# l90lpa/fv3-jedi-linearmodel

Hardware: AMD Instinct MI355X
Metric: column-updates/s per TL+AD dyn step (higher is better)
Workload: dtype f64; 1 GPU; C192L127 hydrostatic TL+AD, six cube faces dealt over 1 GPU(s) (6 per rank), table-driven exchange (221184 columns per GPU), k_split=2 n_split=6 dt=450s nq=4, hord mt/vt/tm/dp/tr=2/2/2/2/2 (sponge: 1/1/1/1 below level 9), kord=17, nord=1; columns_per_gpu=221184

## Files before the change

### fv3_jedi_linearmodel_amd/csrc/dycore.h

```cpp
#pragma once
#include "../../include/fv3lm.h"
#include "stages.h"
#include "column.h"
#include "exchange.h"
#include "nh.h"
#include "nh_ad.h"
#include "tpfused.h"
#include "tpad.h"
#include "tp2.h"
#include "dampt.h"
#include <functional>
#include <map>
#include <memory>
#include <set>
#include <string>
#include <vector>

namespace fv3 {

#ifdef FV3LM_HOST_EMUL
inline void* dev_alloc(size_t n) { void* p = std::calloc(n ? n : 1, 1); return p; }
inline void dev_free(void* p) { std::free(p); }
inline void dev_zero(Exec&, void* p, size_t n) { std::memset(p, 0, n); }
inline void dev_copy(Exec&, void* d, const void* s, size_t n) { std::memcpy(d, s, n); }
inline void h2d(Exec&, void* d, const void* s, size_t n) { std::memcpy(d, s, n); }
inline void d2h(Exec&, void* d, const void* s, size_t n) { std::memcpy(d, s, n); }
inline void dev_sync(Exec&) {}
#else
#define HIPCHK(x) do { hipError_t e_ = (x); if (e_ != hipSuccess) { char b_[320]; std::snprintf(b_, sizeof b_, "HIP error '%s' at %s:%d (%s)", hipGetErrorString(e_), __FILE__, __LINE__, #x); set_sticky(b_); } } while (0)
inline void* dev_alloc(size_t n) {
  void* p = nullptr;
  if (!sticky_error().empty()) return nullptr;
  const hipError_t e = hipMalloc(&p, n ? n : 8);
  if (e != hipSuccess) { char b_[200]; std::snprintf(b_, sizeof b_, "hipMalloc of %zu bytes failed: %s", n, hipGetErrorString(e)); set_sticky(b_); (void)hipGetLastError(); return nullptr; }
  HIPCHK(hipMemset(p, 0, n ? n : 8));
  return p;
}
inline void dev_free(void* p) { if (p) (void)hipFree(p); }
__global__ void __launch_bounds__(256) k_zero16(double2* p, size_t n2) {
  const size_t stride = (size_t)gridDim.x * 256;
  for (size_t i = (size_t)blockIdx.x * 256 + threadIdx.x; i < n2; i += stride) p[i] = make_double2(0., 0.);
}
inline void dev_zero(Exec& ex, void* p, size_t n) {
  if (n >= ((size_t)1 << 20) && ((uintptr_t)p & 7) == 0) {
    char* q = (char*)p;
    if ((uintptr_t)q & 15) { HIPCHK(hipMemsetAsync(q, 0, 8, ex.stream)); q += 8; n -= 8; }
    const size_t n2 = n / 16, want = (n2 + 255) / 256;
    hipLaunchKernelGGL(k_zero16, dim3((unsigned)(want < 8192 ? want : 8192)), dim3(256), 0, ex.stream, (double2*)q, n2);
    if (n & 15) HIPCHK(hipMemsetAsync(q + n2 * 16, 0, n & 15, ex.stream));
    return;
  }
  HIPCHK(hipMemsetAsync(p, 0, n, ex.stream));
}
inline void dev_copy(Exec& ex, void* d, const void* s, size_t n) { HIPCHK(hipMemcpyAsync(d, s, n, hipMemcpyDeviceToDevice, ex.stream)); }
inline void h2d(Exec& ex, void* d, const void* s, size_t n) { HIPCHK(hipMemcpyAsync(d, s, n, hipMemcpyHostToDevice, ex.stream)); HIPCHK(hipStreamSynchronize(ex.stream)); }
inline void d2h(Exec& ex, void* d, const void* s, size_t n) { HIPCHK(hipMemcpyAsync(d, s, n, hipMemcpyDeviceToHost, ex.stream)); HIPCHK(hipStreamSynchronize(ex.stream)); }
inline void dev_sync(Exec& ex) { HIPCHK(hipStreamSynchronize(ex.stream)); }
#endif

struct Arena {
  double* t = nullptr; double* p = nullptr; size_t cap = 0, used = 0;
  void measure() { cap = (size_t)1 << 56; t = p = (double*)(uintptr_t)4096; used = 0; }
  void init(size_t ndoubles) { cap = ndoubles; t = (double*)dev_alloc(cap * 8); p = (double*)dev_alloc(cap * 8); used = 0; }
  void destroy() { dev_free(t); dev_free(p); t = p = nullptr; }
  Fld take(size_t n, int nk) {
    if (used + n > cap) { set_sticky("internal sizing error: field arena overflow"); Fld f; f.t = t; f.p = p; f.nk = nk; return f; }
    Fld f; f.t = t + used; f.p = p + used; f.nk = nk; used += n; return f;
  }
};

typedef fv3lm_options Options;

inline bool resolve_level(const Options& o, int k, int npz, LevelParams& lp) {
  int hord_m = o.hord_mt, hord_t = o.hord_tm, hord_v = o.hord_vt, hord_p = o.hord_dp;
  int nord_k = o.nord, nord_v = (2 > o.nord) ? o.nord : 2;
  double d2_divg = (0.20 > o.d2_bg) ? o.d2_bg : 0.20;
  double damp_vt = o.do_vort_damp ? o.vtdm4 : 0.;
  int nord_w = nord_v, nord_t = nord_v;
  double damp_w = damp_vt, damp_t = damp_vt, d_con_k = o.d_con;
  if (npz == 1 || o.n_sponge < 0) {
    d2_divg = o.d2_bg;
  } else if (k == 1) {
    nord_k = 0;
    if (0.01 < o.d2_bg) d2_divg = (o.d2_bg < o.d2_bg_k1) ? o.d2_bg_k1 : o.d2_bg;
    else if (0.01 < o.d2_bg_k1) d2_divg = o.d2_bg_k1;
    else d2_divg = 0.01;
    nord_w = 0; damp_w = d2_divg;
    if (o.do_vort_damp) { nord_v = 0; damp_vt = 0.5 * d2_divg; }
    d_con_k = 0.;
  } else {
    const int max1 = (2 < o.n_sponge - 1) ? o.n_sponge - 1 : 2;
    if (k == max1 && o.d2_bg_k2 > 0.01) {
      nord_k = 0; d2_divg = (o.d2_bg < o.d2_bg_k2) ? o.d2_bg_k2 : o.d2_bg;
      nord_w = 0; damp_w = d2_divg;
      if (o.do_vort_damp) { nord_v = 0; damp_vt = 0.5 * d2_divg; }
      d_con_k = 0.;
    } else {
      const int max2 = (3 < o.n_sponge) ? o.n_sponge : 3;
      if (k == max2 && o.d2_bg_k2 > 0.05) {
        nord_k = 0; d2_divg = (o.d2_bg < 0.2 * o.d2_bg_k2) ? 0.2 * o.d2_bg_k2 : o.d2_bg;
        nord_w = 0; damp_w = d2_divg; d_con_k = 0.;
      }
    }
  }
  int hmp = o.hord_mt_pert, htp = o.hord_tm_pert, hvp = o.hord_vt_pert, hpp = o.hord_dp_pert;
  int nord_k_pert = o.nord_pert;
  int nord_v_pert = (2 > o.nord_pert) ? o.nord_pert : 2;
  double damp_vt_pert = o.do_vort_damp_pert ? o.vtdm4_pert : 0.;
  double d2_divg_pert = (0.20 > o.d2_bg_pert) ? o.d2_bg_pert : 0.20;
  const int nord_t_pert = nord_v_pert; const double damp_t_pert = damp_vt_pert;
  if (k <= o.n_sponge_pert) {
    nord_k_pert = 0;
    if (k <= o.n_sponge_pert - 1) {
      if (o.hord_ks_traj) { hord_m = o.hord_mt_ks_traj; hord_t = o.hord_tm_ks_traj; hord_v = o.hord_vt_ks_traj; hord_p = o.hord_dp_ks_traj; }
      if (o.hord_ks_pert) { hmp = o.hord_mt_ks_pert; htp = o.hord_tm_ks_pert; hvp = o.hord_vt_ks_pert; hpp = o.hord_dp_ks_pert; }
    }
    const double kfac = (k == 1) ? o.d2_bg_k1_pert : (k == 2) ? o.d2_bg_k2_pert : o.d2_bg_ks_pert;
    double d2p;
    if (0.01 < o.d2_bg_pert) d2p = (o.d2_bg_pert < kfac) ? kfac : o.d2_bg_pert;
    else if (0.01 < kfac) d2p = kfac;
    else d2p = 0.01;
    d2_divg_pert = d2p;
    if (o.do_vort_damp_pert) { nord_v_pert = 0; damp_vt_pert = 0.5 * d2p; }
  }
  lp.hord_mt = hmp; lp.hord_vt = hvp; lp.hord_tm = htp; lp.hord_dp = hpp; lp.hord_tr = o.hord_tr_pert;
  lp.hord_tm_g = o.hord_tm_pert;
  lp.hord_mt_t = hord_m; lp.hord_vt_t = hord_v; lp.hord_tm_t = hord_t; lp.hord_dp_t = hord_p; lp.hord_tr_t = o.hord_tr; lp.hord_tm_g_t = o.hord_tm;
  lp.nord = nord_k; lp.nord_v = nord_v; lp.nord_w = nord_w; lp.nord_t = nord_t; lp.nord_v_pert = nord_v_pert;
  lp.d2_divg = d2_divg; lp.damp_vt = damp_vt; lp.damp_w = damp_w; lp.damp_t = damp_t; lp.d_con = d_con_k;
  lp.damp_vt_pert = damp_vt_pert;
  lp.split_damp = o.split_damp ? 1 : 0; lp.nord_t_pert = nord_t_pert; lp.damp_t_pert = damp_t_pert;
  lp.dddmp = o.dddmp; lp.d4_bg = o.d4_bg;
  if (o.split_damp) { lp.nord_p = nord_k_pert; lp.d2_divg_p = d2_divg_pert; lp.dddmp_p = o.dddmp_pert; lp.d4_bg_p = o.d4_bg_pert; }
  else { lp.nord_p = nord_k; lp.d2_divg_p = d2_divg; lp.dddmp_p = o.dddmp; lp.d4_bg_p = o.d4_bg; }
  return true;
}

struct Op {
  std::string group;
  std::function<void(Exec&, int)> fn;
  bool accum = false;
  unsigned modes = 7u;
  std::vector<double*> ad_in, ad_out;
  std::vector<int> ad_in_slot;
  std::function<void(unsigned, Rect)> set_wmask;
  std::vector<Rect> ad_out_rect;
  std::vector<double*> ad_store;
  std::string name;
  bool global = false;
  Op() = default;
  Op(std::string g_, std::function<void(Exec&, int)> f_, bool acc_ = false) : group(std::move(g_)), fn(std::move(f_)), accum(acc_) {}
};
typedef std::vector<Op> Program;
struct Progs {
  std::vector<Program> c; const int* cur = nullptr;
  Program& now() { return c[(size_t)(*cur < 0 ? 0 : *cur)]; }
  operator Program&() { return now(); }
  void clear() { now().clear(); }
};

struct Dycore {
  Geom g{}; Options opt; Exec ex; Ctx ctx{};
  double bdt = 0; int n_split = 1, k_split = 1, nq = 0;
// ... 210 lines not shown
      for (size_t n = 0; n < it->ad_in.size(); ++n) {
        double* q_ = it->ad_in[n];
        if (!inA(q_) || written.count(q_)) continue;
        const char* skip = std::getenv("FV3LM_AD_WRITE_SKIP");
        const bool skipped = skip && ("," + std::string(skip) + ",").find("," + it->name + ",") != std::string::npos;
        if (std::getenv("FV3LM_AD_WRITE_LIST") && it->set_wmask && !skipped && !zero.count(q_)) std::fprintf(stderr, "write-mode %s input %d\n", it->name.c_str(), it->ad_in_slot[n]);
        if (!off && !skipped && it->set_wmask && n < it->ad_in_slot.size() && !zero.count(q_)) {
          w |= 1u << it->ad_in_slot[n];
          grow((everywhere.count(q_) || !prod.count(q_)) ? whole : prod[q_]);
        }
        else zero.insert(q_);
        written.insert(q_);
      }
      if (it->set_wmask) it->set_wmask(w, wr);
    }
    std::vector<std::pair<double*, size_t>> out;
    for (double* q_ : zero) {
      const size_t n = size.count(q_) ? size[q_] : 0;
      if (!n) { set_sticky("internal error: adjoint plan met an unregistered work array"); continue; }
      if (!out.empty() && out.back().first + out.back().second == q_) out.back().second += n; else out.push_back({q_, n});
    }
    if (std::getenv("FV3LM_AD_WRITE_LIST")) { size_t tot = 0; for (auto& z_ : out) tot += z_.second; std::fprintf(stderr, "plan_adjoint: %zu work adjoints cleared per pass (%zu ranges, %.1f field-equivalents of %zu in the arena)\n", zero.size(), out.size(), double(tot) / double(n3 ? n3 : 1), size.size()); }
    return out;
  }
  std::vector<std::pair<double*, size_t>> acoustic_zero;

  void build_tp(Program& P, const char* grp, const std::string& pre, Fld q, Fld crx, Fld cry, Fld xfx, Fld yfx, Fld rax,
                Fld ray, Fld mx, Fld my, Fld mass, int hsel, int dsel, bool use_mass, Fld fx, Fld fy, int nk = 0, const Fld* acc4 = nullptr) {
    const int is = g.is(), ie = g.ie(), js = g.js(), je = g.je(), isd = g.isd(), ied = g.ied(), jsd = g.jsd(), jed = g.jed(), npz = nk ? nk : g.npz;
    const char* fenv = std::getenv("FV3LM_TP_FUSED");
    const bool fused = !(fenv && fenv[0] == '0');
    const char* aenv = std::getenv("FV3LM_TP_AD_FUSED");
    const int adf = !fused ? 0 : aenv ? (aenv[0] == '0' ? 0 : aenv[0] == '1' ? 1 : 2) : 2;
    const bool own_fo = adf == 0, own_mid = adf < 2;
    Fld fy2 = own_mid ? W((pre + "_fy2").c_str(), npz) : fy, q_i = own_mid ? W((pre + "_qi").c_str(), npz) : fx;
    Fld fx2 = own_mid ? W((pre + "_fx2").c_str(), npz) : fx, q_j = own_mid ? W((pre + "_qj").c_str(), npz) : fy;
    Fld fxo = own_fo ? W((pre + "_fxo").c_str(), npz) : fx2, fyo = own_fo ? W((pre + "_fyo").c_str(), npz) : fy2;
    const size_t first_op = P.size();
    auto ppm_y = [&](Fld qq, Fld out, Rect r, int cdir) {
      TpPpmY_<false> a; a.in[0] = qq; a.in[1] = cry; a.out[0] = out; a.k1 = npz; a.hsel = hsel;
      if (!g.face) { a.orect[0] = r; add(P, grp, a); return; }
      const int npy = g.ny + 1;
      a.orect[0] = isect(r, R(r.i0, r.i1, 4, npy - 3));
      TpPpmY_<true> e; e.in[0] = qq; e.in[1] = cry; e.out[0] = out; e.k1 = npz; e.hsel = hsel; e.cdir = cdir;
      std::vector<TpPpmY_<true>> ev;
      for (const Rect& er : {isect(r, R(r.i0, r.i1, r.j0, 3)), isect(r, R(r.i0, r.i1, npy - 2, r.j1))}) if (!is_empty(er)) { e.orect[0] = er; ev.push_back(e); }
      add_multi(P, grp, ev);
      if (!is_empty(a.orect[0])) add(P, grp, a);
    };
    auto ppm_x = [&](Fld qq, Fld out, Rect r, int cdir) {
      TpPpmX_<false> a; a.in[0] = qq; a.in[1] = crx; a.out[0] = out; a.k1 = npz; a.hsel = hsel;
      if (!g.face) { a.orect[0] = r; add(P, grp, a); return; }
      const int npx = g.nx + 1;
      a.orect[0] = isect(r, R(4, npx - 3, r.j0, r.j1));
      TpPpmX_<true> e; e.in[0] = qq; e.in[1] = crx; e.out[0] = out; e.k1 = npz; e.hsel = hsel; e.cdir = cdir;
      std::vector<TpPpmX_<true>> ev;
      for (const Rect& er : {isect(r, R(r.i0, 3, r.j0, r.j1)), isect(r, R(npx - 2, r.i1, r.j0, r.j1))}) if (!is_empty(er)) { e.orect[0] = er; ev.push_back(e); }
      add_multi(P, grp, ev);
      if (!is_empty(a.orect[0])) add(P, grp, a);
    };
    ppm_y(q, fy2, R(isd, ied, js, je + 1), 2);
    TpQi b; b.in[0] = q; b.in[1] = fy2; b.in[2] = yfx; b.in[3] = ray; b.out[0] = q_i; b.orect[0] = R(isd, ied, js, je); b.k1 = npz;
    add(P, grp, b);
    const size_t o1a = P.size();
    ppm_x(q_i, fxo, R(is, ie + 1, js, je), 0);
    const size_t o1b = P.size();
    ppm_x(q, fx2, R(is, ie + 1, jsd, jed), 1);
    TpQj e; e.in[0] = q; e.in[1] = fx2; e.in[2] = xfx; e.in[3] = rax; e.out[0] = q_j; e.orect[0] = R(is, ie, jsd, jed); e.k1 = npz;
    add(P, grp, e);
    const size_t o2a = P.size();
    ppm_y(q_j, fyo, R(is, ie, js, je + 1), 0);
    const size_t o2b = P.size();
    Fld d2b{};
    if (dsel != DAMP_NONE) {
      d2b = W((pre + "_d2b").c_str(), npz);
      TpD2D h; h.in[0] = q; h.out[0] = d2b; h.orect[0] = R(is - 1, ie + 1, js - 1, je + 1); h.k1 = npz; h.dsel = dsel; h.use_mass = use_mass; h.hsel = hsel;
      add_face(P, grp, h, 1);
    }
    bool any_split = false;
    for (int k = 0; k < npz && k < (int)lev_host.size(); ++k) any_split = any_split || level_split(lev_host[k], hsel, dsel);
    TpFlux t; t.in[0] = fxo; t.in[1] = fx2; t.in[2] = mx; t.in[3] = fyo; t.in[4] = fy2; t.in[5] = my;
    t.in[6] = (dsel != DAMP_NONE) ? q : Fld{}; t.in[7] = d2b; t.in[8] = use_mass ? mass : Fld{};
    for (int n = 6; n < 9; ++n) if (!t.in[n].t) t.in[n].nk = npz;
    t.out[0] = fx; t.out[1] = fy; t.orect[0] = R(is, ie + 1, js, je); t.orect[1] = R(is, ie, js, je + 1); t.k1 = npz;
    t.dsel = dsel; t.use_mass = use_mass; t.hsel = hsel;
    const size_t o3 = P.size();
    add(P, grp, t);
    if (any_split && !fused) set_sticky("split_hord / split_damp need the fused fv_tp_2d (unset FV3LM_TP_FUSED)");
    if (fused) {
      size_t d2_op = P.size();
      for (size_t n = first_op; n < P.size(); ++n) if (P[n].name == "TpD2" || P[n].name == "TpD2e") d2_op = n;
      for (size_t n = first_op; n < P.size(); ++n) if (!(P[n].name == "TpD2" || P[n].name == "TpD2e")) P[n].modes = 1u << MODE_AD;
      (void)d2_op;
      TpFusedArgs a; a.q = q; a.crx = crx; a.cry = cry; a.xfx = xfx; a.yfx = yfx; a.rax = rax; a.ray = ray; a.mx = mx; a.my = my;
      a.mass = use_mass ? mass : Fld{}; a.d2b = d2b; a.fx = fx; a.fy = fy;
      a.fy2 = fy2; a.q_i = q_i; a.fxo = fxo; a.fx2 = fx2; a.q_j = q_j; a.fyo = fyo;
      a.hsel = hsel; a.dsel = dsel; a.use_mass = use_mass ? 1 : 0; a.nk = npz;
      a.do_acc = 0; a.store_fo = own_fo ? 1 : 0; a.store_mid = own_mid ? 1 : 0;
      if (acc4) { a.acx = acc4[0]; a.acy = acc4[1]; a.amfx = acc4[2]; a.amfy = acc4[3]; }
      Ctx* cp = &ctx;
      Op op{grp, [a, cp](Exec& e, int mode) { run_tp_fused(e, mode, a, *cp); }};
      op.modes = (1u << MODE_NL) | (1u << MODE_TL);
      op.name = "TpFused";
      for (const Fld* f_ : {&a.q, &a.crx, &a.cry, &a.xfx, &a.yfx, &a.rax, &a.ray, &a.mx, &a.my, &a.mass, &a.d2b}) if (f_->p) op.ad_in.push_back(f_->p);
      for (const Fld* f_ : {&a.fx, &a.fy, &a.fy2, &a.q_i, &a.fxo, &a.fx2, &a.q_j, &a.fyo, &a.acx, &a.acy, &a.amfx, &a.amfy}) if (f_->p) op.ad_out.push_back(f_->p);
      P.push_back(op);
      if (any_split) {
        if (dsel != DAMP_NONE) {
          Fld d2t = W((pre + "_d2t").c_str(), npz);
          bool nord2 = false;
          for (int k = 0; k < npz && k < (int)lev_host.size(); ++k) { int n_; double d_; damp_of(lev_host[k], dsel, n_, d_, false); nord2 = nord2 || (n_ == 2 && d_ > 1.e-4 && level_split(lev_host[k], hsel, dsel)); }
          const size_t n0 = P.size();
          TpD2D h; h.in[0] = q; h.out[0] = d2t; h.orect[0] = R(is - 1, ie + 1, js - 1, je + 1); h.k1 = npz; h.dsel = dsel; h.use_mass = use_mass; h.hsel = hsel; h.traj = 1;
          if (nord2) {
            Fld d2a = W((pre + "_d2a").c_str(), npz);
            TpD2D h1 = h; h1.out[0] = d2a; h1.orect[0] = R(is - 2, ie + 2, js - 2, je + 2); h1.pass = 1;
            add_face(P, grp, h1, 2);
            h.in[0] = d2a;
          }
          add_face(P, grp, h, 1);
          for (size_t n = n0; n < P.size(); ++n) {
            auto f = P[n].fn;
            P[n].fn = [f](Exec& e, int) { f(e, MODE_NL); };
            P[n].modes = (1u << MODE_NL) | (1u << MODE_TL); P[n].ad_in.clear(); P[n].ad_in_slot.clear(); P[n].ad_out.clear(); P[n].ad_out_rect.clear(); P[n].set_wmask = nullptr;
          }
          a.d2b_t = d2t;
        }
        Op tr{grp, [a, cp](Exec& e, int mode) { run_tp_fused(e, mode, a, *cp, true); }};
        tr.modes = (1u << MODE_NL) | (1u << MODE_TL); tr.name = "TpFusedTraj";
        P.push_back(tr);
      }
      if (adf > 0) {
        if (adf == 2) { for (size_t n = first_op; n < o3; ++n) if (!(P[n].name == "TpD2" || P[n].name == "TpD2e")) P[n].modes = 0; }
        else { for (size_t n = o1a; n < o1b; ++n) P[n].modes = 0; for (size_t n = o2a; n < o2b; ++n) P[n].modes = 0; }
        P[o3].modes = 0;
        if (dsel != DAMP_NONE) {
          TpDamp dm; dm.in[0] = q; dm.in[1] = d2b; dm.in[2] = use_mass ? mass : Fld{};
          for (int n = 1; n < 3; ++n) if (!dm.in[n].t) dm.in[n].nk = npz;
          dm.out[0] = fx; dm.out[1] = fy; dm.orect[0] = R(is, ie + 1, js, je); dm.orect[1] = R(is, ie, js, je + 1); dm.k1 = npz;
          dm.dsel = dsel; dm.use_mass = use_mass; dm.hsel = hsel;
          add(P, grp, dm); P.back().modes = 1u << MODE_AD;
        }
        Op ad{grp, [a, cp, adf](Exec& e, int) { if (adf == 2) run_tp_ad(e, a, *cp); else run_tp_outer_ad(e, a, *cp); }};
        ad.modes = 1u << MODE_AD; ad.name = adf == 2 ? "TpAd" : "TpOuter";
        ad.ad_out = {fx.p, fy.p}; ad.ad_out_rect = {R(is, ie + 1, js, je), R(is, ie, js, je + 1)};
        if (adf == 2) ad.ad_in = {q.p, crx.p, cry.p, xfx.p, yfx.p, rax.p, ray.p, mx.p, my.p};
        else { ad.ad_store = {q_i.p, q_j.p, fx2.p, fy2.p}; ad.ad_in = {crx.p, cry.p, mx.p, my.p}; }
        P.push_back(ad);
      }
    }
  }
  void build_a2b(Program& P, const char* grp, const std::string& pre, Fld q, Fld qb, int nk) {
    const int is = g.is(), ie = g.ie(), js = g.js(), je = g.je();
    Fld qx = W((pre + "_qx").c_str(), nk), qy = W((pre + "_qy").c_str(), nk);
    const int npx = g.nx + 1, npy = g.ny + 1;
    A2bA_<false> a; a.in[0] = q; a.out[0] = qx; a.out[1] = qy; a.k1 = nk;
    A2bB_<false> b; b.in[0] = qx; b.in[1] = qy; b.in[2] = Fld{}; b.out[0] = qb; b.k1 = nk;
    if (!g.face) {
      a.orect[0] = R(is, ie + 1, js - 2, je + 2); a.orect[1] = R(is - 2, ie + 2, js, je + 1); add(P, grp, a);
      b.orect[0] = R(is, ie + 1, js, je + 1); add(P, grp, b);
      return;
    }
    const Rect qxr = R(is, ie + 1, std::max(1, js - 2), std::min(npy - 1, je + 2)), qyr = R(std::max(1, is - 2), std::min(npx - 1, ie + 2), js, je + 1);
    a.orect[0] = isect(qxr, R(3, npx - 2, qxr.j0, qxr.j1)); a.orect[1] = isect(qyr, R(qyr.i0, qyr.i1, 3, npy - 2));
    const bool a0 = !is_empty(a.orect[0]), a1 = !is_empty(a.orect[1]);
    if (a0 && !a1) a.orect[1] = empty_in(a.orect[0]);
    if (a1 && !a0) a.orect[0] = empty_in(a.orect[1]);
    A2bA_<true> ae; ae.in[0] = q; ae.out[0] = qx; ae.out[1] = qy; ae.k1 = nk;
    std::vector<A2bA_<true>> av;
    for (int e = 0; e < 4; ++e) {
      const Rect r = e == 0 ? isect(qxr, R(1, 2, qxr.j0, qxr.j1)) : e == 1 ? isect(qxr, R(npx - 1, npx, qxr.j0, qxr.j1)) : e == 2 ? isect(qyr, R(qyr.i0, qyr.i1, 1, 2)) : isect(qyr, R(qyr.i0, qyr.i1, npy - 1, npy));
      if (is_empty(r)) continue;
      ae.orect[e < 2 ? 0 : 1] = r; ae.orect[e < 2 ? 1 : 0] = empty_in(r); av.push_back(ae);
    }
    add_multi(P, grp, av);
    if (a0 || a1) add(P, grp, a);
    const Rect qbr = R(is, ie + 1, js, je + 1);
    b.orect[0] = isect(qbr, R(3, npx - 2, 3, npy - 2));
    A2bB_<true> be; be.in[0] = qx; be.in[1] = qy; be.in[2] = q; be.out[0] = qb; be.k1 = nk;
    std::vector<A2bB_<true>> bv;
    for (int e = 0; e < 4; ++e) {
      const Rect r = isect(qbr, e == 0 ? R(1, npx, 1, 2) : e == 1 ? R(1, npx, npy - 1, npy) : e == 2 ? R(1, 2, 3, npy - 2) : R(npx - 1, npx, 3, npy - 2));
      if (is_empty(r)) continue;
      be.orect[0] = r; bv.push_back(be);
    }
    add_multi(P, grp, bv);
    if (!is_empty(b.orect[0])) add(P, grp, b);
  }

  void build_acoustic();
  bool init(int nx, int ny, int npz, int ntile, int face, int nq_, double bdt_, int n_split_, int k_split_, const Options& o,
            const double* const* metrics_host, double da_min, double da_min_c, const double* phis_host, int nface = 0, const int* ij0 = nullptr);
  void destroy();

  void run_group(Progs& P, const char* group, int mode, bool skip_accum = false);
  void zero_work_adjoint() { dev_zero(ex, work.p, work.used * 8); }
  void dyn_core(int mode);
};

inline void Dycore::run_group(Progs& PS, const char* group, int mode, bool skip_accum) {
  const bool all = (group == nullptr) || (group[0] == 0);
  ex.skip_accum = skip_accum;
  const int nc = (int)PS.c.size();
  auto take = [&](const Op& op) { return (all || op.group == group) && !(mode != MODE_AD && skip_accum && op.accum) && ((op.modes >> mode) & 1u); };
  if (nc == 1) {
    set_class(0);
    const Program& P = PS.c[0];
    if (mode != MODE_AD) { for (const Op& op : P) if (take(op)) { if (op.global) set_class(-1); op.fn(ex, mode); if (op.global) set_class(0); } }
    else for (auto it = P.rbegin(); it != P.rend(); ++it) if (take(*it)) { if (it->global) set_class(-1); it->fn(ex, mode); if (it->global) set_class(0); }
    set_class(-1);
    ex.skip_accum = false;
    return;
  }
  std::vector<std::vector<size_t>> gl(nc);
  for (int c = 0; c < nc; ++c) for (size_t n = 0; n < PS.c[c].size(); ++n) if (PS.c[c][n].global) gl[c].push_back(n);
  for (int c = 1; c < nc; ++c) if (gl[c].size() != gl[0].size()) { set_sticky("internal error: the tile classes' programs hold different exchange sequences"); ex.skip_accum = false; return; }
  const size_t nseg = gl[0].size() + 1;
  auto seg = [&](int c, size_t sg, size_t& a, size_t& b) { a = sg == 0 ? 0 : gl[c][sg - 1] + 1; b = sg < gl[c].size() ? gl[c][sg] : PS.c[c].size(); };
  if (mode != MODE_AD) {
    for (size_t sg = 0; sg < nseg; ++sg) {
      for (int c = 0; c < nc; ++c) { size_t a, b; seg(c, sg, a, b); set_class(c); for (size_t n = a; n < b; ++n) if (take(PS.c[c][n])) PS.c[c][n].fn(ex, mode); }
      if (sg < gl[0].size()) { const Op& op = PS.c[0][gl[0][sg]]; set_class(-1); if (take(op)) op.fn(ex, mode); }
    }
  } else {
    for (size_t sg = nseg; sg-- > 0;) {
      if (sg < gl[0].size()) { const Op& op = PS.c[0][gl[0][sg]]; set_class(-1); if (take(op)) op.fn(ex, mode); }
      for (int c = 0; c < nc; ++c) { size_t a, b; seg(c, sg, a, b); set_class(c); for (size_t n = b; n-- > a;) if (take(PS.c[c][n])) PS.c[c][n].fn(ex, mode); }
    }
  }
  set_class(-1);
  ex.skip_accum = false;
}

inline void Dycore::set_class(int c) {
  cur_cls = c;
  g.ntile = ntile_all; g.i0 = 1; g.j0 = 1; ctx.m = m_all; ex.cls_off = 0;
  if (c >= 0 && c < (int)classes.size()) {
    const TileClass& k = classes[(size_t)c];
    g.ntile = k.n; g.i0 = k.i0; g.j0 = k.j0;
    const size_t op = (size_t)k.t0 * g.plane;
    Metrics& M = ctx.m;
    const double** slots[] = {&M.area, &M.rarea, &M.rarea_c, &M.dx, &M.dy, &M.dxa, &M.dya, &M.dxc, &M.dyc, &M.rdx, &M.rdy, &M.rdxa,
                              &M.rdya, &M.rdxc, &M.rdyc, &M.cosa, &M.sina, &M.rsina, &M.cosa_u, &M.cosa_v, &M.cosa_s, &M.sina_u,
                              &M.sina_v, &M.rsin_u, &M.rsin_v, &M.rsin2, &M.f0, &M.fC, &M.del6_u, &M.del6_v, &M.divg_u, &M.divg_v};
    for (auto sl : slots) *sl += op;
    for (int n = 1; n <= 9; ++n) { M.sin_sg[n] += op; M.cos_sg[n] += op; }
    if (M.edge) M.edge += (size_t)k.t0 * 4 * g.pj;
    if (M.ecorner) M.ecorner += (size_t)k.t0 * 12;
    ex.cls_off = op;
  }
  ctx.g = g;
}

inline bool Dycore::init(int nx, int ny, int npz, int ntile, int face, int nq_, double bdt_, int n_split_, int k_split_,
                         const Options& o, const double* const* metrics_host, double da_min, double da_min_c,
                         const double* phis_host, int nface, const int* ij0) {
  g.tx = nx; g.ty = ny; g.nx = (face && nface > 0) ? nface : nx; g.ny = (face && nface > 0) ? nface : ny;
  g.ng = 3; g.npz = npz; g.ntile = ntile; g.face = face ? 1 : 0; g.pi = nx + 2 * g.ng + 1; g.pj = ny + 2 * g.ng + 1;
  g.plane = g.pi * g.pj; g.i0 = g.j0 = 1;
  ntile_all = ntile;
  classes.clear();
  for (int t = 0; t < ntile; ++t) {
    const int i0 = ij0 ? ij0[2 * t] : 1, j0 = ij0 ? ij0[2 * t + 1] : 1;
    if (i0 < 1 || j0 < 1 || i0 + nx - 1 > g.nx || j0 + ny - 1 > g.ny) { err = "tile window outside its face"; return false; }
    if (!classes.empty() && classes.back().i0 == i0 && classes.back().j0 == j0) classes.back().n++;
    else classes.push_back(TileClass{t, 1, i0, j0});
  }
  subtile = face && !(g.tx == g.nx && g.ty == g.ny);
  if (!subtile) for (const TileClass& k : classes) if (k.i0 != 1 || k.j0 != 1) { err = "a whole-face tile starts at (1, 1)"; return false; }
  if (subtile && g.nx != g.ny) { err = "cube faces are square"; return false; }
  opt = o; bdt = bdt_; n_split = n_split_; k_split = k_split_; nq = nq_;
  if (nx < 8 || ny < 8 || npz < 1) { err = "tile too small (need nx,ny >= 8)"; return false; }
  if (!face && ntile != 1) { err = "ntile > 1 needs face = 1 (whole cube faces); face = 0 is the single doubly-periodic tile"; return false; }
  if (face && nx != ny) { err = "cube faces (and their tiles) are square: nx must equal ny"; return false; }
  if (ntile < 1) { err = "ntile < 1"; return false; }
  nh = !o.hydrostatic;
  if (o.nord_pert > 1 || o.nord_pert < 0) { err = "nord_pert in {0,1} only (the divergence damping whose tangent / adjoint is taken; the trajectory's nord may be 2 or 3 with split_damp)"; return false; }
  if (o.nord > 3 || o.nord < 0) { err = "nord in 0..3 only"; return false; }
  if (!o.split_damp) {
    if (o.nord != o.nord_pert || o.dddmp != o.dddmp_pert || o.d2_bg != o.d2_bg_pert || o.d4_bg != o.d4_bg_pert || (o.do_vort_damp != 0) != (o.do_vort_damp_pert != 0) ||
        o.vtdm4 != o.vtdm4_pert || o.d2_bg_k1 != o.d2_bg_k1_pert || o.d2_bg_k2 != o.d2_bg_k2_pert) {
      err = "split_damp = 0 but the trajectory's damping options (nord, dddmp, d2_bg, d4_bg, do_vort_damp, vtdm4, d2_bg_k1, d2_bg_k2) differ from the *_pert ones: set split_damp = 1 "
            "(fv_arrays_tlmadm.F90:76) or hand over equal values (run_setup_pert, fv_control_tlmadm.F90:220-229)";
      return false;
    }
  } else {
    if (o.nord == 0 && o.nord_pert > 0) { err = "split_damp: nord = 0 with nord_pert > 0 -- c_sw computes divg_d only for the trajectory's nord > 0 (sw_core_tlm.F90: IF (nord .GT. 0) divergence_corner), the perturbation's damping would read an undefined array"; return false; }
    if (nh && o.nord > 1) { err = "non-hydrostatic with a trajectory nord > 1: the w / height damping would need the tangent of del6_vt_flux with nord 2 (sw_core_tlm.F90:1713-1726), not built"; return false; }
  }
  if (nh && npz < 3) { err = "non-hydrostatic solver needs npz >= 3"; return false; }
  if (!nh && npz < 2) { err = "hydrostatic vertical remap: the column map (edge values of cs_profile / scalar_profile) needs npz >= 2"; return false; }
  if (nh && !(o.a_imp > 0.5)) { err = "non-hydrostatic: a_imp must be > 0.5 (semi-implicit solver; the reference's a_imp <= 0.5 Riemann-invariant solver is not built)"; return false; }
  for (int kd : {o.kord_tm_pert, o.kord_mt_pert, o.kord_wz_pert, o.kord_tr_pert})
    if ((kd < 0 ? -kd : kd) <= 16) { err = "kord_*_pert: only |kord| > 16 (the linear profile, the one the TL/AD reference differentiates) is built"; return false; }
  for (int kd : {o.kord_tm, o.kord_mt, o.kord_wz, o.kord_tr}) {
    const int ak = kd < 0 ? -kd : kd;
    if (ak <= 16 && !(ak >= 8 && ak <= 15)) { err = "kord_tm/kord_mt/kord_wz/kord_tr: the linear profile (|kord| > 16) or, for the trajectory, the limited profiles 8 .. 15 of cs_profile / scalar_profile (not 16, not ppm_profile's 7 and below)"; return false; }
    if (ak <= 16 && npz < 6) { err = "kord: limited trajectory profiles need npz >= 6"; return false; }
  }
  lev_host.resize(npz + 1);
  for (int k = 1; k <= npz; ++k) {
    resolve_level(o, k, npz, lev_host[k - 1]);
    const LevelParams& l = lev_host[k - 1];
    for (int h : {l.hord_mt, l.hord_vt, l.hord_tm, l.hord_dp, l.hord_tr, l.hord_tm_g})
      if (h != 1 && h != 2 && h != 333) { err = "perturbation hord must be 1, 2 or 333 (the schemes the TL/AD reference implements)"; return false; }
    for (int h : {l.hord_mt_t, l.hord_vt_t, l.hord_tm_t, l.hord_dp_t, l.hord_tr_t, l.hord_tm_g_t})
// ... 541 lines not shown
```

Baseline: 183,700 column-updates/s.

## Fuse A-to-B grid interpolation into one LDS-tiled kernel for NL/TL/AD

Replaces the multi-kernel a2b path (separate x/y line interpolation kernels writing qx/qy work arrays, then edge and corner kernels) with a single tiled kernel that stages q, qx and qy in LDS per 64xH block and writes qb directly. A hand-written adjoint kernel gathers contributions through LDS, using dual-number seeded weights near face edges and corners. This removes intermediate global arrays and several launches, at the cost of heavy LDS use per block (lower occupancy) and slow per-point dual evaluations at face boundaries. It is enabled by default and can be turned off with an environment variable.

```diff
diff --git a/fv3_jedi_linearmodel_amd/csrc/a2b.h b/fv3_jedi_linearmodel_amd/csrc/a2b.h
--- /dev/null
+++ b/fv3_jedi_linearmodel_amd/csrc/a2b.h
@@ -0,0 +1,245 @@
+#pragma once
+#include "tpfused.h"
+
+namespace fv3 {
+
+struct A2bArgs {
+  Fld q, qb;
+  int nk = 0;
+  unsigned wmask = 0;
+};
+FV3LM_LINK void run_a2b(Exec& ex, int mode, const A2bArgs& a0, const Ctx& c);
+inline bool a2b_fused_enabled() { const char* e = std::getenv("FV3LM_A2B_FUSED"); return !(e && e[0] == '0'); }
+}
+
+#if !defined(FV3LM_SPLIT_BUILD) || defined(FV3LM_IMPL_A2B)
+namespace fv3 {
+#ifndef FV3LM_A2B_H
+#define FV3LM_A2B_H 16
+#endif
+#ifndef FV3LM_A2B_WAVES
+#define FV3LM_A2B_WAVES 8
+#endif
+constexpr int A2B_W = 64, A2B_H = FV3LM_A2B_H;
+constexpr int A2B_PQ = A2B_W + 6, A2B_PX = A2B_W + 1, A2B_RQ = A2B_H + 6, A2B_RY = A2B_H + 1;
+constexpr int A2B_OQ = 0, A2B_OX = A2B_OQ + A2B_PQ * A2B_RQ, A2B_OY = A2B_OX + A2B_PX * A2B_RQ, A2B_NT = A2B_OY + A2B_PQ * A2B_RY;
+template <class T> constexpr size_t a2b_lds_bytes() { return (size_t)A2B_NT * sizeof(T); }
+constexpr int A2B_OW = A2B_W + 7, A2B_OH = A2B_H + 7;
+constexpr int A2B_PB = A2B_OW + 5, A2B_RB = A2B_OH + 5;
+constexpr int A2B_OB = 0, A2B_OXA = A2B_OB + A2B_PB * A2B_RB, A2B_OYA = A2B_OXA + A2B_PB * A2B_OH, A2B_NAD = A2B_OYA + A2B_OW * A2B_RB;
+constexpr size_t a2b_lds_bytes_ad() { return (size_t)A2B_NAD * 8; }
+static_assert(a2b_lds_bytes<Dual>() <= 80 * 1024, "a2b tangent block: LDS over 80 KB (fewer than two blocks per CU)");
+static_assert(a2b_lds_bytes<double>() <= 40 * 1024, "a2b nonlinear block: LDS over 40 KB (fewer than four blocks per CU)");
+static_assert(a2b_lds_bytes_ad() <= 53 * 1024, "a2b adjoint block: LDS over 53 KB (fewer than three blocks per CU)");
+
+template <int NWV, class F>
+DEV void a2b_sweep(int tid, int nc, int nr, const F& f) {
+#ifdef FV3LM_HOST_EMUL
+  (void)tid;
+  for (int r = 0; r < nr; ++r) for (int x = 0; x < nc; ++x) f(x, r);
+#else
+  const int lane = tid & 63, wv = __builtin_amdgcn_readfirstlane(tid >> 6);
+  if (lane < nc) for (int r = wv; r < nr; r += NWV) f(lane, r);
+  const int hc = nc - 64;
+  if (hc > 0) for (int e = tid; e < hc * nr; e += 64 * NWV) f(64 + e % hc, e / hc);
+#endif
+}
+
+template <class T>
+struct A2bLds {
+  const T *q, *qx, *qy; int qi0, qj0, yj0;
+  static constexpr unsigned want = ~0u;
+  template <int M> HD T in(int i, int j, int = 0) const {
+    if (M == 0) return qx[(j - qj0) * A2B_PX + (i - qi0 - 3)];
+    if (M == 1) return qy[(j - yj0) * A2B_PQ + (i - qi0)];
+    return q[(j - qj0) * A2B_PQ + (i - qi0)];
+  }
+};
+struct A2bSeed {
+  int m, si, sj;
+  static constexpr unsigned want = ~0u;
+  template <int M> HD Dual in(int i, int j, int = 0) const { return Dual(0., (M == m && i == si && j == sj) ? 1. : 0.); }
+};
+struct A2bSeedLine { int s; HD Dual operator()(int k) const { return Dual(0., k == s ? 1. : 0.); } };
+template <class D>
+HD double a2b_wline(int m, int n1, int s, const D& d) { return A2bA_<true>::line<Dual>(true, m, n1, A2bSeedLine{s}, d).d; }
+HD double a2b_wcorner(const Ctx& c, int tile, int i, int j, int k, int m, int si, int sj) {
+  const A2bB_<true> b{}; Dual o; b.eval<Dual>(A2bSeed{m, si, sj}, c, tile, i, j, k, &o); return o.d;
+}
+
+template <class T, int NWV>
+DEV void a2b_block(const A2bArgs& a, const Ctx& c, int tile, int k, int bx, int by, T* lds, int tid) {
+  const Geom& g = c.g;
+  const bool face = g.face != 0;
+  const int npx = g.nx + 1, npy = g.ny + 1, pi = g.pi;
+  const int is = g.is(), ie = g.ie(), js = g.js(), je = g.je();
+  const int I0 = is + bx * A2B_W, J0 = js + by * A2B_H;
+  const int I1 = (I0 + A2B_W - 1 < ie) ? I0 + A2B_W - 1 : ie + 1, J1 = (J0 + A2B_H - 1 < je) ? J0 + A2B_H - 1 : je + 1;
+  const int nc = I1 - I0 + 1, nr = J1 - J0 + 1;
+  const size_t pq = (size_t)(tile * a.q.nk + k - 1) * g.plane, pb = (size_t)(tile * a.qb.nk + k - 1) * g.plane;
+  T* const Q = lds + A2B_OQ; T* const QX = lds + A2B_OX; T* const QY = lds + A2B_OY;
+  const size_t qbase = pq + (size_t)g.idx(I0 - 3, J0 - 3);
+  a2b_sweep<NWV>(tid, nc + 5, nr + 5, [&](int x, int r) { Q[r * A2B_PQ + x] = TpfIO<T>::ld(a.q, qbase + (size_t)r * pi + x); });
+  TPF_SYNC();
+  a2b_sweep<NWV>(tid, nc, nr + 5, [&](int x, int r) {
+    const int i = I0 + x, j = J0 - 3 + r;
+    if (face && (j < 1 || j > npy - 1)) return;
+    const T* row = Q + r * A2B_PQ; const int o = I0 - 3;
+    QX[r * A2B_PX + x] = A2bA_<true>::line<T>(face, i, npx, [row, o](int m) { return row[m - o]; }, MetX{c.m.dxa, c, tile, j});
+  });
+  a2b_sweep<NWV>(tid, nc + 5, nr, [&](int x, int r) {
+    const int i = I0 - 3 + x, j = J0 + r;
+    if (face && (i < 1 || i > npx - 1)) return;
+    const T* col = Q + x; const int o = J0 - 3;
+    QY[r * A2B_PQ + x] = A2bA_<true>::line<T>(face, j, npy, [col, o](int m) { return col[(m - o) * A2B_PQ]; }, MetY{c.m.dya, c, tile, i});
+  });
+  TPF_SYNC();
+  const A2bLds<T> acc{Q, QX, QY, I0 - 3, J0 - 3, J0};
+  const size_t obase = pb + (size_t)g.idx(I0, J0);
+  a2b_sweep<NWV>(tid, nc, nr, [&](int x, int r) {
+    const int i = I0 + x, j = J0 + r;
+    T o;
+    if (face && (i <= 2 || i >= npx - 1 || j <= 2 || j >= npy - 1)) { const A2bB_<true> b{}; b.eval<T>(acc, c, tile, i, j, k, &o); }
+    else { const A2bB_<false> b{}; b.eval<T>(acc, c, tile, i, j, k, &o); }
+    TpfIO<T>::st(a.qb, obase + (size_t)r * pi + x, o);
+  });
+}
+
+template <int NWV>
+DEV void a2b_block_ad(const A2bArgs& a, const Ctx& c, int tile, int k, int bx, int by, int nbx, int nby, bool store, double* lds, int tid) {
+  const Geom& g = c.g;
+  const bool face = g.face != 0;
+  const int npx = g.nx + 1, npy = g.ny + 1;
+  const int is = g.is(), ie = g.ie(), js = g.js(), je = g.je();
+  const int C0 = bx == 0 ? g.isd() : is + bx * A2B_W, C1 = bx == nbx - 1 ? g.ied() + 1 : is + bx * A2B_W + A2B_W - 1;
+  const int R0 = by == 0 ? g.jsd() : js + by * A2B_H, R1 = by == nby - 1 ? g.jed() + 1 : js + by * A2B_H + A2B_H - 1;
+  const int nc = C1 - C0 + 1, nr = R1 - R0 + 1;
+  const size_t pq = (size_t)(tile * a.q.nk + k - 1) * g.plane, pb = (size_t)(tile * a.qb.nk + k - 1) * g.plane;
+  double* const B = lds + A2B_OB; double* const XA = lds + A2B_OXA; double* const YA = lds + A2B_OYA;
+  auto b_at = [&](int i, int j) -> double { return B[(j - (R0 - 2)) * A2B_PB + (i - (C0 - 2))]; };
+  a2b_sweep<NWV>(tid, nc + 5, nr + 5, [&](int x, int r) {
+    const int i = C0 - 2 + x, j = R0 - 2 + r;
+    B[r * A2B_PB + x] = (i >= is && i <= ie + 1 && j >= js && j <= je + 1) ? a.qb.p[pb + (size_t)g.idx(i, j)] : 0.;
+  });
+  TPF_SYNC();
+  a2b_sweep<NWV>(tid, nc + 5, nr, [&](int x, int r) {
+    const int m = C0 - 2 + x, rr = R0 + r;
+    double s = 0.;
+    if (m >= is && m <= ie + 1 && !(face && (rr < 1 || rr > npy - 1))) {
+      if (face && (m == 1 || m == npx || rr <= 4 || rr >= npy - 4)) {
+        for (int jp = rr - 2; jp <= rr + 3; ++jp) { const double bv = b_at(m, jp); if (bv != 0.) s += a2b_wcorner(c, tile, m, jp, k, 0, m, rr) * bv; }
+      } else s = (0.5 * A2) * b_at(m, rr - 1) + (0.5 * A1) * b_at(m, rr) + (0.5 * A1) * b_at(m, rr + 1) + (0.5 * A2) * b_at(m, rr + 2);
+    }
+    XA[r * A2B_PB + x] = s;
+  });
+  a2b_sweep<NWV>(tid, nc, nr + 5, [&](int x, int r) {
+    const int ii = C0 + x, n = R0 - 2 + r;
+    double s = 0.;
+    if (n >= js && n <= je + 1 && !(face && (ii < 1 || ii > npx - 1))) {
+      if (face && (n == 1 || n == npy || ii <= 4 || ii >= npx - 4)) {
+        for (int ip = ii - 2; ip <= ii + 3; ++ip) { const double bv = b_at(ip, n); if (bv != 0.) s += a2b_wcorner(c, tile, ip, n, k, 1, ii, n) * bv; }
+      } else s = (0.5 * A2) * b_at(ii - 1, n) + (0.5 * A1) * b_at(ii, n) + (0.5 * A1) * b_at(ii + 1, n) + (0.5 * A2) * b_at(ii + 2, n);
+    }
+    YA[r * A2B_OW + x] = s;
+  });
+  TPF_SYNC();
+  auto xa = [&](int m, int j) -> double { return XA[(j - R0) * A2B_PB + (m - (C0 - 2))]; };
+  auto ya = [&](int i, int n) -> double { return YA[(n - (R0 - 2)) * A2B_OW + (i - C0)]; };
+  const bool st = store;
+  a2b_sweep<NWV>(tid, nc, nr, [&](int x, int r) {
+    const int i = C0 + x, j = R0 + r;
+    const bool reach = i >= is - 2 && i <= ie + 2 && j >= js - 2 && j <= je + 2;
+    if (!reach && !st) return;
+    double s = 0.;
+    if (reach) {
+      const bool ex = face && (i <= 4 || i >= npx - 4), ey = face && (j <= 4 || j >= npy - 4);
+      if (!ex && !ey) {
+        const double w[4] = {B2, B1, B1, B2};
+#pragma unroll
+        for (int d = 0; d < 4; ++d) { s += w[d] * xa(i - 1 + d, j); s += w[d] * ya(i, j - 1 + d); }
+      } else {
+        if (ex) {
+          const int m0 = i - 2 > is ? i - 2 : is, m1 = i + 3 < ie + 1 ? i + 3 : ie + 1;
+          const MetX d{c.m.dxa, c, tile, j};
+          for (int m = m0; m <= m1; ++m) { const double v = xa(m, j); if (v != 0.) s += a2b_wline(m, npx, i, d) * v; }
+        } else {
+          const double w[4] = {B2, B1, B1, B2};
+          for (int d = 0; d < 4; ++d) s += w[d] * xa(i - 1 + d, j);
+        }
+        if (ey) {
+          const int n0 = j - 2 > js ? j - 2 : js, n1 = j + 3 < je + 1 ? j + 3 : je + 1;
+          const MetY d{c.m.dya, c, tile, i};
+          for (int n = n0; n <= n1; ++n) { const double v = ya(i, n); if (v != 0.) s += a2b_wline(n, npy, j, d) * v; }
+        } else {
+          const double w[4] = {B2, B1, B1, B2};
+          for (int d = 0; d < 4; ++d) s += w[d] * ya(i, j - 1 + d);
+        }
+        if (i <= 3 || i >= npx - 3 || j <= 3 || j >= npy - 3) {
+          for (int jp = j - 1; jp <= j + 2; ++jp)
+            for (int ip = i - 1; ip <= i + 2; ++ip) {
+              if (!(ip == 1 || ip == 2 || ip == npx - 1 || ip == npx || jp == 1 || jp == 2 || jp == npy - 1 || jp == npy)) continue;
+              const double bv = b_at(ip, jp);
+              if (bv != 0.) s += a2b_wcorner(c, tile, ip, jp, k, 2, i, j) * bv;
+            }
+        }
+      }
+    }
+    double* qa = a.q.p + pq + (size_t)g.idx(i, j);
+    if (st) *qa = s; else *qa += s;
+  });
+}
+
+inline void a2b_grid(const Geom& g, int& nbx, int& nby) { nbx = (g.tx + A2B_W - 1) / A2B_W; nby = (g.ty + A2B_H - 1) / A2B_H; }
+
+#ifndef FV3LM_HOST_EMUL
+template <class T, int NWV>
+__global__ void __launch_bounds__(64 * NWV) k_a2b(A2bArgs a, Ctx c) {
+  extern __shared__ __attribute__((aligned(16))) unsigned char a2b_lds[];
+  int bx = blockIdx.x, by = blockIdx.y; xcd_block(gridDim.x, gridDim.y, bx, by);
+  a2b_block<T, NWV>(a, c, blockIdx.z / a.nk, 1 + blockIdx.z % a.nk, bx, by, reinterpret_cast<T*>(a2b_lds), threadIdx.x);
+}
+template <int NWV>
+__global__ void __launch_bounds__(64 * NWV) k_a2b_ad(A2bArgs a, Ctx c, int store) {
+  extern __shared__ __attribute__((aligned(16))) unsigned char a2b_lds[];
+  int bx = blockIdx.x, by = blockIdx.y; xcd_block(gridDim.x, gridDim.y, bx, by);
+  a2b_block_ad<NWV>(a, c, blockIdx.z / a.nk, 1 + blockIdx.z % a.nk, bx, by, gridDim.x, gridDim.y, store != 0, reinterpret_cast<double*>(a2b_lds), threadIdx.x);
+}
+#endif
+
+inline double a2b_bytes(const A2bArgs& a, const Geom& g, int mode, bool store) {
+  const double pts = double(g.tx + 1) * (g.ty + 1) * g.ntile * a.nk;
+  return 8. * pts * (mode == MODE_NL ? 2. : mode == MODE_TL ? 4. : store ? 2. : 3.);
+}
+
+FV3LM_LINK void run_a2b(Exec& ex, int mode, const A2bArgs& a0, const Ctx& c) {
+  A2bArgs a = a0;
+  a.q = ex.sh(a.q); a.qb = ex.sh(a.qb);
+  const bool store = mode == MODE_AD && (a.wmask & 1u) && !ex.no_wmask;
+  int nbx, nby; a2b_grid(c.g, nbx, nby);
+  ex.mark_begin("A2b", mode == MODE_AD ? ".ad" : mode == MODE_TL ? ".tl" : ".nl", a2b_bytes(a, c.g, mode, store));
+#ifdef FV3LM_HOST_EMUL
+  std::vector<double> lds((a2b_lds_bytes<Dual>() > a2b_lds_bytes_ad() ? a2b_lds_bytes<Dual>() : a2b_lds_bytes_ad()) / 8 + 1);
+  for (int z = 0; z < c.g.ntile * a.nk; ++z)
+    for (int by = 0; by < nby; ++by)
+      for (int bx = 0; bx < nbx; ++bx) {
+        if (mode == MODE_AD) a2b_block_ad<1>(a, c, z / a.nk, 1 + z % a.nk, bx, by, nbx, nby, store, lds.data(), 0);
+        else if (mode == MODE_TL) a2b_block<Dual, 1>(a, c, z / a.nk, 1 + z % a.nk, bx, by, reinterpret_cast<Dual*>(lds.data()), 0);
+        else a2b_block<double, 1>(a, c, z / a.nk, 1 + z % a.nk, bx, by, lds.data(), 0);
+      }
+#else
+  const dim3 grid(nbx, nby, c.g.ntile * a.nk), block(64 * FV3LM_A2B_WAVES);
+  static bool attr = false;
+  if (!attr) {
+    if (hipFuncSetAttribute((const void*)k_a2b<Dual, FV3LM_A2B_WAVES>, hipFuncAttributeMaxDynamicSharedMemorySize, (int)a2b_lds_bytes<Dual>()) != hipSuccess) set_sticky("hipFuncSetAttribute(k_a2b) failed");
+    attr = true;
+  }
+  if (mode == MODE_AD) hipLaunchKernelGGL((k_a2b_ad<FV3LM_A2B_WAVES>), grid, block, a2b_lds_bytes_ad(), ex.stream, a, c, store ? 1 : 0);
+  else if (mode == MODE_TL) hipLaunchKernelGGL((k_a2b<Dual, FV3LM_A2B_WAVES>), grid, block, a2b_lds_bytes<Dual>(), ex.stream, a, c);
+  else hipLaunchKernelGGL((k_a2b<double, FV3LM_A2B_WAVES>), grid, block, a2b_lds_bytes<double>(), ex.stream, a, c);
+#endif
+  ex.mark_end();
+  ex.launches++;
+}
+
+}
+#endif
diff --git a/fv3_jedi_linearmodel_amd/csrc/dycore.h b/fv3_jedi_linearmodel_amd/csrc/dycore.h
--- a/fv3_jedi_linearmodel_amd/csrc/dycore.h
+++ b/fv3_jedi_linearmodel_amd/csrc/dycore.h
@@ -9,6 +9,7 @@
 #include "tpad.h"
 #include "tp2.h"
 #include "dampt.h"
+#include "a2b.h"
 #include <functional>
 #include <map>
 #include <memory>
@@ -525,6 +526,16 @@
   }
   void build_a2b(Program& P, const char* grp, const std::string& pre, Fld q, Fld qb, int nk) {
     const int is = g.is(), ie = g.ie(), js = g.js(), je = g.je();
+    if (a2b_fused_enabled()) {
+      A2bArgs a; a.q = q; a.qb = qb; a.nk = nk;
+      auto ap = std::make_shared<A2bArgs>(a); Ctx* cp = &ctx;
+      Op op{grp, [ap, cp](Exec& e, int mode) { run_a2b(e, mode, *ap, *cp); }};
+      op.ad_in = {q.p}; op.ad_in_slot = {0}; op.ad_out = {qb.p}; op.ad_out_rect = {R(is, ie + 1, js, je + 1)};
+      op.set_wmask = [ap](unsigned w, Rect) { ap->wmask = w; };
+      op.name = "A2b";
+      P.push_back(op);
+      return;
+    }
     Fld qx = W((pre + "_qx").c_str(), nk), qy = W((pre + "_qy").c_str(), nk);
     const int npx = g.nx + 1, npy = g.ny + 1;
     A2bA_<false> a; a.in[0] = q; a.out[0] = qx; a.out[1] = qy; a.k1 = nk;
diff --git a/fv3_jedi_linearmodel_amd/csrc/tu_a2b.cpp b/fv3_jedi_linearmodel_amd/csrc/tu_a2b.cpp
--- /dev/null
+++ b/fv3_jedi_linearmodel_amd/csrc/tu_a2b.cpp
@@ -0,0 +1,2 @@
+#define FV3LM_IMPL_A2B
+#include "a2b.h"
```

Result: slower. 180,000 column-updates/s (median of 2 runs) (-2.0%).
